# ade-ma/LibRedio

Measured on AMD Instinct MI355X. Metric: MSamples/s through FIR+FFT+resample chain, higher is better.
Workload: dtype f32

## Files before the change

__graft_entry__.py:

```python
import os
import subprocess
import sys

ROOT = os.path.dirname(os.path.abspath(__file__))
sys.path.insert(0, ROOT)


def build() -> None:
    import libredio_amd
    libredio_amd.build()
    libredio_amd.lib()
    libredio_amd.kisslib()
    import oracle
    oracle.build()
    oracle.lib()
    libredio_amd.samplerate_lib()
    subprocess.check_call(["make", "-C", os.path.join(ROOT, "tests", "emu"), "-s"])
    subprocess.check_call(["make", "-C", os.path.join(ROOT, "tests", "cpp"), "-s"])
    subprocess.check_call(["make", "-C", os.path.join(ROOT, "tests", "stub"), "-s"])
    subprocess.check_call(["make", "-C", os.path.join(ROOT, "tests", "cpp_src"), "-s"])
    subprocess.check_call(["make", "-C", os.path.join(ROOT, "tests", "emu_fftr"), "-s"])
    subprocess.check_call(["make", "-C", os.path.join(ROOT, "tests", "cpp_fftr"), "-s"])
    subprocess.check_call(["make", "-C", os.path.join(ROOT, "tests", "emu_ovsave_real"), "-s"])
    subprocess.check_call(["make", "-C", os.path.join(ROOT, "tests", "cpp_ovsave_real"), "-s"])
    subprocess.check_call(["make", "-C", os.path.join(ROOT, "tests", "emu_pspec"), "-s"])
    subprocess.check_call(["make", "-C", os.path.join(ROOT, "tests", "cpp_pspec"), "-s"])
    subprocess.check_call(["make", "-C", os.path.join(ROOT, "tests", "emu_pspec_u8"), "-s"])
    subprocess.check_call(["make", "-C", os.path.join(ROOT, "tests", "cpp_pspec_u8"), "-s"])
    subprocess.check_call(["make", "-C", os.path.join(ROOT, "tests", "emu_pspec_real"), "-s"])
    subprocess.check_call(["make", "-C", os.path.join(ROOT, "tests", "cpp_pspec_real"), "-s"])
    subprocess.check_call(["make", "-C", os.path.join(ROOT, "tests", "emu_pfb_pspec"), "-s"])
    subprocess.check_call(["make", "-C", os.path.join(ROOT, "tests", "cpp_pfb_pspec"), "-s"])
    subprocess.check_call(["make", "-C", os.path.join(ROOT, "tests", "emu_taps"), "-s"])
    subprocess.check_call(["make", "-C", os.path.join(ROOT, "tests", "emu_route"), "-s"])
    subprocess.check_call(["make", "-C", os.path.join(ROOT, "tests", "emu_sched"), "-s"])


def smoke() -> None:
    import numpy as np
    import torch
    import libredio_amd as R
    import oracle as O

    assert torch.cuda.is_available(), "smoke() needs a HIP device"
    torch.cuda.set_device(0)
    n = 8 * 1024 * 5 + 126
    taps = R.dsputils.lpf_corrected(127, 0.08)
    x = R.synth_iq(0x5EED0002, 0, n)
    xh = O.synth_iq(0x5EED0002, 0, n)
    assert np.array_equal(x.cpu().numpy().view(np.uint32), xh.view(np.uint32)), "device/host synthetic input differ"
    for fused in (True, False):
        chain = R.Chain(taps, 5, 1024, fused=fused)
        assert chain.is_fused
        got = chain(x).cpu().numpy()
        want = O.chain_fir_fft(xh, taps, 5, 1024, fused=fused)
        assert got.shape == want.shape == (8, 1024)
        assert np.array_equal(got.view(np.uint32), want.view(np.uint32)), f"chain (fused={fused}) differs from the oracle"
    print("smoke ok: fused FIR(127,/5)->FFT1024 chain is bit-identical to the oracle on 8 blocks")


if __name__ == "__main__":
    build()
    if len(sys.argv) > 1 and sys.argv[1] == "smoke":
        smoke()
```

libredio_amd/csrc/chain_v4.hip:

```cpp
#ifndef REDIO_EXP_CHAIN_NT
#define REDIO_EXP_CHAIN_NT 3
#endif
#ifndef REDIO_EXP_SEAM
#define REDIO_EXP_SEAM 15
#endif
#include "fir_core.h"
#include "fft_wave.h"
#include "redio_internal.h"
#include "../../include/redio.h"
#include <type_traits>

namespace redio {

typedef float v4f_t __attribute__((ext_vector_type(4)));

constexpr int chain_gcd(int a, int b) { return b == 0 ? a : chain_gcd(b, a % b); }

template <int N, typename F>
__device__ __forceinline__ void static_for4(F &&f)
{
    if constexpr (N > 0) {
        static_for4<N - 1>(f);
        f(std::integral_constant<int, N - 1>{});
    }
}

template <int K, int D, bool FUSED, int WPS, int CH, bool FIR_ONLY, bool TWP, bool IN_U8, bool PF2, bool RES, int SCH>
__device__ __forceinline__ void chain_v4_body(const float2 *__restrict__ x, const float *__restrict__ taps,
                                              const float2 *__restrict__ tw, float2 *__restrict__ out,
                                              long nblocks, long blocks_per_wave, long wave, unsigned long long *dbg, long dbg_cap)
{
    unsigned long long t0c = 0, t0r = 0;
    if (dbg) { t0c = __builtin_amdgcn_s_memtime(); t0r = __builtin_amdgcn_s_memrealtime(); }
    constexpr int R = 4;
    using G = FirGeomV<K, D, R>;
    constexpr int SUB_OUT = 64 * R;
    constexpr int SUB_NEW = SUB_OUT * D;
    constexpr int HALO = G::tile_in(SUB_OUT) - SUB_NEW;
    static_assert(HALO % 2 == 0 && SUB_NEW % 128 == 0 && 4 * SUB_OUT == 1024, "geometry");
    constexpr int HALO_V = HALO / 2;
    constexpr int NLD = SUB_NEW / 2 / 64;
    static_assert(HALO_V <= 64, "the halo moves with one instruction per lane");
    extern __shared__ __attribute__((aligned(16))) char smem[];
    v4f_t *xs4 = reinterpret_cast<v4f_t *>(smem);
    float2 *ex = reinterpret_cast<float2 *>(smem);

    const int lane = threadIdx.x;
    const long b0 = wave * blocks_per_wave;
    if (b0 >= nblocks) return;
    const long b1 = (b0 + blocks_per_wave < nblocks) ? b0 + blocks_per_wave : nblocks;
    const long nsub = 4 * (b1 - b0);
    typename std::conditional<RES, FirTapsResident<K>, FirNoResidentTaps>::type rtaps;
    if constexpr (RES) fir_taps_resident_load(rtaps, taps);
    using pair_t = typename std::conditional<IN_U8, unsigned, v4f_t>::type;
    [[maybe_unused]] const pair_t *src0 = (IN_U8 ? reinterpret_cast<const pair_t *>(reinterpret_cast<const unsigned *>(x) + b0 * 512 * (long)D)
                                : reinterpret_cast<const pair_t *>(x + b0 * 1024 * (long)D)) + lane;
    auto samples = [](pair_t w) -> v4f_t {
        if constexpr (IN_U8) return v4f_t{i2f(w & 255u), i2f((w >> 8) & 255u), i2f((w >> 16) & 255u), i2f(w >> 24)};
        else return w;
    };

    constexpr bool HOIST = (REDIO_EXP_SEAM & 1) != 0, BUF = PF2 || (REDIO_EXP_SEAM & 2) != 0, EARLY = (REDIO_EXP_SEAM & 4) != 0,
                   PRO = (REDIO_EXP_SEAM & 8) != 0;
    auto slot = [](int p) { return G::lds_index(2 * p) / 2; };
    constexpr int HSTR = G::LSTR / 2;
    static_assert((SUB_NEW / 2) % HSTR == 0, "a sub-tile is a whole number of lane strides");
    constexpr int HALO_DELTA = G::lds_index(SUB_NEW) / 2;
    constexpr int PER0 = G::PADN == 0 ? 1 : HSTR / chain_gcd(64, HSTR), PER = PER0 < NLD ? PER0 : NLD;
    constexpr int PARK_STEP = G::lds_index(2 * 64 * PER) / 2;
    static_assert(PER == NLD || (64 * PER) % HSTR == 0, "park slots repeat with period PER");
    auto halo_slots = [&](int lf, int &src, int &dst) {
        dst = slot(lf);
        if constexpr (EARLY) src = dst + (lf < HALO_V ? HALO_DELTA : 0);
        else src = slot(SUB_NEW / 2 + lf);
    };
    [[maybe_unused]] int park4[PER], hsrc4 = 0, hdst4 = 0;
    if constexpr (HOIST) {
        static_for4<PER>([&](auto I) { park4[I.value] = slot(HALO_V + lane + 64 * I.value); });
        halo_slots(lane, hsrc4, hdst4);
    }

    pair_t pre[NLD], pre2[PF2 ? NLD : 1];
    constexpr unsigned PB = sizeof(pair_t);
    constexpr int NT_LD = (REDIO_EXP_CHAIN_NT & 1) ? 2 : 0, NT_ST = (REDIO_EXP_CHAIN_NT & 2) ? 2 : 0;
    typedef unsigned v4u_t __attribute__((ext_vector_type(4)));
    typedef unsigned v2u_t __attribute__((ext_vector_type(2)));
    [[maybe_unused]] __amdgpu_buffer_rsrc_t ri, ro;
    if constexpr (BUF) {
        static_assert(!PF2 || !IN_U8, "PF2: cf32 input");
        const char *xb = reinterpret_cast<const char *>(x) + b0 * (512 * (long)D) * PB;
        ri = __builtin_amdgcn_make_buffer_rsrc(const_cast<char *>(xb), 0, (int)((HALO_V + nsub * (SUB_NEW / 2)) * PB), 0x00020000);
        ro = __builtin_amdgcn_make_buffer_rsrc(out + b0 * 1024, 0, (int)((b1 - b0) * 8192), 0x00020000);
    }
    [[maybe_unused]] auto buf_load = [&](unsigned vo, unsigned so, auto policy) -> pair_t {
        if constexpr (IN_U8) return __builtin_amdgcn_raw_buffer_load_b32(ri, vo, so, decltype(policy)::value);
        else return __builtin_bit_cast(v4f_t, __builtin_amdgcn_raw_buffer_load_b128(ri, vo, so, decltype(policy)::value));
    };
    auto fetch_to = [&](pair_t(&dst)[NLD], long j) {
        if constexpr (BUF) {
            const unsigned sub = (unsigned)((HALO_V + j * (SUB_NEW / 2)) * PB);
            const unsigned vo = PB * (unsigned)lane + (PF2 ? sub : 0u), so = PF2 ? 0u : sub;
            static_for4<NLD>([&](auto I) {
                constexpr unsigned off = 64u * PB * I.value, imm = off % 4096u;
                dst[I.value] = buf_load(vo + imm, so + (off - imm), std::integral_constant<int, NT_LD>{});
                if constexpr (!PF2) __builtin_amdgcn_sched_barrier(0);
            });
        } else {
            const pair_t *src = src0 + HALO_V + j * (SUB_NEW / 2);
#if REDIO_EXP_CHAIN_NT & 1
            static_for4<NLD>([&](auto I) { dst[I.value] = __builtin_nontemporal_load(src + 64 * I.value); });
#else
            static_for4<NLD>([&](auto I) { dst[I.value] = src[64 * I.value]; });
#endif
        }
    };
    auto park_from = [&](pair_t(&from)[NLD]) {
#if REDIO_EXP_ABLATE == 3
#pragma unroll
        for (int i = 0; i < NLD; ++i) { pair_t keep = from[i]; asm volatile("" : : "v"(keep)); }
#else
        static_for4<NLD>([&](auto I) {
            constexpr int i = I.value;
            if constexpr (HOIST) xs4[park4[i % PER] + (i / PER) * PARK_STEP] = samples(from[i]);
            else xs4[G::lds_index(HALO + 2 * (lane + 64 * i)) / 2] = samples(from[i]);
        });
#endif
    };
    [[maybe_unused]] auto store_block = [&](const float2(&a)[16], long blk, int ln) {
        if constexpr (BUF) {
            const unsigned so = (unsigned)(blk * 8192);
            static_for4<16>([&](auto I) {
                constexpr unsigned k0 = I.value / 4, k1 = I.value % 4;
                const float2 v = a[k1 + 4 * k0];
                __builtin_amdgcn_raw_buffer_store_b64(v2u_t{__builtin_bit_cast(unsigned, v.x), __builtin_bit_cast(unsigned, v.y)}, ro,
                                                      8u * (unsigned)ln + (512u * k1 + 2048u * (k0 & 1)), so + 4096u * (k0 >> 1), NT_ST);
            });
        } else fft1kn_store_spectrum(a, out + (b0 + blk) * 1024, ln);
    };

    static_assert(SCH == 0 || (!PF2 && !FIR_ONLY && TWP && WPS == 2), "the block schedules: the transforming product forms");
    constexpr int EXH_OFF = G::lds_elems(SUB_OUT) > FFT1KN_LDS ? G::lds_elems(SUB_OUT) : FFT1KN_LDS;
    constexpr int T12_OFF = EXH_OFF + (SCH == 2 ? FFT1KN_HALF_LDS : 0);
    constexpr bool TABLE = (PF2 || SCH != 0) && !FIR_ONLY;
    static_assert(!TABLE || (T12_OFF + 64) * sizeof(float2) <= 160 * 1024 / 8 - 480, "within the request of chain_v4_lds at two waves per SIMD");
    auto table_index = [](int l) {
        const int k4 = l / 15, i = l % 15;
        return i < 3 ? 64 * k4 * (i + 1) : 16 * (k4 + 4 * ((i - 3) / 3)) * ((i - 3) % 3 + 1);
    };
    Fft1knTw34 t34;
    [[maybe_unused]] float2 one = make_float2(0.f, 0.f);
    if constexpr (PRO) {
        pair_t head;
        if constexpr (BUF) head = buf_load(PB * (unsigned)lane, 0u, std::integral_constant<int, 0>{});
        else head = src0[0];
        fetch_to(pre, 0);
        [[maybe_unused]] float2 twv = make_float2(0.f, 0.f);
        if constexpr (TABLE) twv = tw[table_index(lane < 60 ? lane : 0)];
        if (!FIR_ONLY && TWP) fft1kn_load_tw34(t34, lane, tw);
        if constexpr (SCH != 0) one = tw[0];
        xs4[slot(lane)] = samples(head);
        if constexpr (TABLE) ex[T12_OFF + lane] = twv;
        park_from(pre);
        wave_lds_fence();
    } else {
        if (lane < HALO_V) {
            if constexpr (BUF) xs4[slot(lane)] = samples(buf_load(PB * (unsigned)lane, 0u, std::integral_constant<int, 0>{}));
            else xs4[slot(lane)] = samples(src0[0]);
        }
        if constexpr (TABLE)
            if (lane < 60) ex[T12_OFF + lane] = tw[table_index(lane)];
        fetch_to(pre, 0);
        park_from(pre);
        wave_lds_fence();
        if (!FIR_ONLY && TWP) fft1kn_load_tw34(t34, lane, tw);
        if constexpr (SCH != 0) one = tw[0];
    }
    if constexpr (SCH != 0) asm volatile("" : "+v"(one.x), "+v"(one.y));

    float2 a[16];
    if constexpr (!(PRO && SCH == 1)) {
#pragma unroll
        for (int i = 0; i < 16; ++i) a[i] = make_float2(0.f, 0.f);
    }
    constexpr int NCH = fir_num_chunks<K, D, R, CH>();
    struct Seam { int lf, hs, hd; v4f_t halo; };
    auto fir = [&](Seam &s, float2(&acc)[R], auto &&hook) {
        s.lf = lane, s.hs = hsrc4, s.hd = hdst4, s.halo = v4f_t{0.f, 0.f, 0.f, 0.f};
        if constexpr (!HOIST) {
            asm volatile("" : "+v"(s.lf));
            if constexpr (EARLY) halo_slots(s.lf, s.hs, s.hd);
        }
        auto hk = [&](auto C) {
            if constexpr (EARLY && decltype(C)::value == NCH - 1) s.halo = xs4[s.hs];
            hook(C);
        };
        if constexpr (RES) fir_lane_v_res<K, D, R, FUSED, CH>(xs4, s.lf, rtaps, acc, hk);
        else fir_lane_v<K, D, R, FUSED, CH>(xs4, s.lf, taps, acc, hk);
    };
    auto halo_read = [&](Seam &s, bool more) {
        if constexpr (!EARLY) {
            if constexpr (!HOIST) halo_slots(s.lf, s.hs, s.hd);
            if (more && s.lf < HALO_V) s.halo = xs4[s.hs];
        }
    };
    auto halo_write = [&](const Seam &s) {
        if constexpr (EARLY) xs4[s.hd] = s.halo;
        else if (s.lf < HALO_V) xs4[HOIST ? s.hd : slot(s.lf)] = s.halo;
    };
    auto transform_lane = [&]() {
        int ln = lane;
        if constexpr (!HOIST) asm volatile("" : "+v"(ln));
        return ln;
    };
    auto step = [&](long j, auto ahead, auto place, pair_t(&req)[NLD], pair_t(&parked)[NLD]) {
        constexpr int AHEAD = decltype(ahead)::value, S = decltype(place)::value;
        const bool more = S >= 0 || j + 1 < nsub;
        if (S >= 0 || j + AHEAD < nsub) fetch_to(req, j + AHEAD);
        float2 acc[R];
#pragma unroll
        for (int r = 0; r < R; ++r) acc[r] = make_float2(0.f, 0.f);
        Seam seam;
        fir(seam, acc, FirNoHook{});
        if (FIR_ONLY) {
            const v4f_t y0 = v4f_t{acc[0].x, acc[0].y, acc[1].x, acc[1].y}, y1 = v4f_t{acc[2].x, acc[2].y, acc[3].x, acc[3].y};
            if constexpr (BUF) {
                const unsigned so = (unsigned)(j * (SUB_OUT * 8));
                __builtin_amdgcn_raw_buffer_store_b128(__builtin_bit_cast(v4u_t, y0), ro, 32u * (unsigned)lane, so, 0);
                __builtin_amdgcn_raw_buffer_store_b128(__builtin_bit_cast(v4u_t, y1), ro, 32u * (unsigned)lane + 16u, so, 0);
            } else {
                v4f_t *y4 = reinterpret_cast<v4f_t *>(out + (b0 * 4 + j) * SUB_OUT) + 2 * lane;
                y4[0] = y0;
                y4[1] = y1;
            }
        } else {
#pragma unroll
            for (int i = 0; i < 12; ++i) a[i] = a[i + 4];
#pragma unroll
            for (int r = 0; r < R; ++r) a[12 + r] = acc[r];
        }
        wave_lds_fence();
        halo_read(seam, more);
        if (!FIR_ONLY && (S == 3 || (S < 0 && (j & 3) == 3))) {
            wave_lds_fence();
            const int ln = transform_lane();
            Fft1knTw12 t12;
            if constexpr (PF2) {
                const float2 *T = ex + T12_OFF + 15 * (ln >> 4);
#pragma unroll
                for (int i = 0; i < 3; ++i) t12.a[i] = T[i];
#pragma unroll
                for (int i = 0; i < 12; ++i) t12.b[i] = T[3 + i];
            } else fft1kn_load_tw12(t12, ln, tw);
            if (!TWP) fft1kn_load_tw34(t34, ln, tw);
            fft1kn_wave_regs<false>(a, ex, tw, t12, t34, ln);
            store_block(a, j >> 2, ln);
            wave_lds_fence();
        }
        if (more) {
            halo_write(seam);
            park_from(parked);
        }
        wave_lds_fence();
    };
    [[maybe_unused]] auto t12_lds = [&](Fft1knTw12 &t12, int ln) {
        const float2 *T = ex + T12_OFF + 15 * (ln >> 4);
#pragma unroll
        for (int i = 0; i < 3; ++i) t12.a[i] = T[i];
#pragma unroll
        for (int i = 0; i < 12; ++i) t12.b[i] = T[3 + i];
    };
    [[maybe_unused]] auto sstep = [&](long j, auto place, bool more_, bool xform_, auto &&hook) {
        constexpr int S = decltype(place)::value;
        const bool more = S < 3 || more_, xform = S == 3 && xform_;
        if (more) fetch_to(pre, j + 1);
        float2 acc[R];
#pragma unroll
        for (int r = 0; r < R; ++r) acc[r] = make_float2(0.f, 0.f);
        Seam seam;
        fir(seam, acc, hook);
#pragma unroll
        for (int r = 0; r < R; ++r) a[4 * S + r] = acc[r];
        wave_lds_fence();
        halo_read(seam, more);
        if (xform) {
            wave_lds_fence();
            const int ln = transform_lane();
            Fft1knTw12 t12;
            t12_lds(t12, ln);
            const float2 one1[1] = {one};
            fft1kn_wave_regs<false>(a, ex, one1, t12, t34, ln);
            store_block(a, j >> 2, ln);
            wave_lds_fence();
        }
        if (more) {
            halo_write(seam);
            park_from(pre);
        }
        wave_lds_fence();
    };
    using S0 = std::integral_constant<int, 0>;
    using S1 = std::integral_constant<int, 1>;
    using S2 = std::integral_constant<int, 2>;
    using S3 = std::integral_constant<int, 3>;
    if constexpr (SCH == 1) {
        const long nb = b1 - b0;
#pragma unroll 1
        for (long blk = 0; blk < nb; ++blk) {
            sstep(4 * blk, S0{}, true, false, FirNoHook{});
            sstep(4 * blk + 1, S1{}, true, false, FirNoHook{});
            sstep(4 * blk + 2, S2{}, true, false, FirNoHook{});
            sstep(4 * blk + 3, S3{}, blk + 1 < nb, true, FirNoHook{});
        }
    } else if constexpr (SCH == 2) {
        const long nb = b1 - b0;
        sstep(0, S0{}, true, false, FirNoHook{});
#pragma unroll 1
        for (long blk = 0;; ++blk) {
            sstep(4 * blk + 1, S1{}, true, false, FirNoHook{});
            sstep(4 * blk + 2, S2{}, true, false, FirNoHook{});
            const bool more = blk + 1 < nb;
            sstep(4 * blk + 3, S3{}, more, !more, FirNoHook{});
            if (!more) break;
            float2 ap[16], u[16];
#pragma unroll
            for (int i = 0; i < 16; ++i) ap[i] = a[i];
            int ln = lane;
            asm volatile("" : "+v"(ln));
            Fft1knTw12 t12;
            float2 *dst = out + (b0 + blk) * 1024;
            auto piece = [&](auto C) {
                fft1kn_wave_piece<decltype(C)::value, false>(ap, u, ex + EXH_OFF, one, ex + T12_OFF + 15 * (ln >> 4), t12, t34, dst, ln);
            };
            sstep(4 * blk + 4, S0{}, true, false, piece);
            if constexpr (NCH < FFT1KN_PIECES)
                static_for4<FFT1KN_PIECES - NCH>([&](auto I) { piece(std::integral_constant<int, NCH + I.value>{}); });
        }
    } else if constexpr (PF2) {
        fetch_to(pre, 1);
        using two = std::integral_constant<int, 2>;
#pragma unroll 1
        for (long j = 0; j < nsub; j += 4) {
            step(j, two{}, std::integral_constant<int, 0>{}, pre2, pre);
            step(j + 1, two{}, std::integral_constant<int, 1>{}, pre, pre2);
            step(j + 2, two{}, std::integral_constant<int, 2>{}, pre2, pre);
            step(j + 3, two{}, std::integral_constant<int, 3>{}, pre, pre2);
        }
    } else {
#pragma unroll 1
        for (long j = 0; j < nsub; ++j) step(j, std::integral_constant<int, 1>{}, std::integral_constant<int, -1>{}, pre, pre);
    }
    if (dbg && lane == 0 && (long)blockIdx.x < dbg_cap) {
        dbg[4 * blockIdx.x] = __builtin_amdgcn_s_memtime() - t0c;
        dbg[4 * blockIdx.x + 1] = __builtin_amdgcn_s_memrealtime() - t0r;
        dbg[4 * blockIdx.x + 2] = t0r;
        unsigned xcc = 0;
        asm volatile("s_getreg_b32 %0, hwreg(HW_REG_XCC_ID)" : "=s"(xcc));
        unsigned hwid = 0;
        asm volatile("s_getreg_b32 %0, hwreg(HW_REG_HW_ID)" : "=s"(hwid));
        dbg[4 * blockIdx.x + 3] = ((unsigned long long)xcc << 32) | hwid;
    }
}

template <int WPS, bool FIR_ONLY, bool TWP, bool PF2, bool RES>
constexpr int chain_v4_sched()
{
    return (WPS == 2 && !FIR_ONLY && TWP && !PF2) ? 1 : 0;
}

template <int K, int D, bool FUSED, int WPS, int CH, bool FIR_ONLY = false, bool TWP = false, bool IN_U8 = false, bool PF2 = false>
__global__ __launch_bounds__(64, WPS) void chain_v4_kernel(const float2 *__restrict__ x, const float *__restrict__ taps,
                                                           const float2 *__restrict__ tw, float2 *__restrict__ out,
                                                           long nblocks, long blocks_per_wave, unsigned long long *dbg, long dbg_cap)
{
    chain_v4_body<K, D, FUSED, WPS, CH, FIR_ONLY, TWP, IN_U8, PF2, true, chain_v4_sched<WPS, FIR_ONLY, TWP, PF2, true>()>(x, taps, tw, out, nblocks, blocks_per_wave, (long)blockIdx.x, dbg, dbg_cap);
}
template <int K, int D, bool FUSED, int WPS, int CH, bool FIR_ONLY = false, bool TWP = false, bool IN_U8 = false, bool PF2 = false>
__global__ __launch_bounds__(64, WPS) void chain_v4_anytaps_kernel(const float2 *__restrict__ x, const float *__restrict__ taps,
                                                                   const float2 *__restrict__ tw, float2 *__restrict__ out,
                                                                   long nblocks, long blocks_per_wave, unsigned long long *dbg, long dbg_cap)
{
    chain_v4_body<K, D, FUSED, WPS, CH, FIR_ONLY, TWP, IN_U8, PF2, false, chain_v4_sched<WPS, FIR_ONLY, TWP, PF2, false>()>(x, taps, tw, out, nblocks, blocks_per_wave, (long)blockIdx.x, dbg, dbg_cap);
}

#ifdef REDIO_MEASURE
template <int K, int D, bool FUSED>
__global__ __launch_bounds__(64, 2) void chain_v4_sched2_kernel(const float2 *__restrict__ x, const float *__restrict__ taps,
                                                                const float2 *__restrict__ tw, float2 *__restrict__ out,
                                                                long nblocks, long blocks_per_wave, unsigned long long *dbg, long dbg_cap)
{
    chain_v4_body<K, D, FUSED, 2, 8, false, true, false, false, true, 2>(x, taps, tw, out, nblocks, blocks_per_wave, (long)blockIdx.x, dbg, dbg_cap);
}
#endif

struct ChainList {
    const float2 *x[REDIO_LIST_MAX];
    float2 *out[REDIO_LIST_MAX];
    long nblocks[REDIO_LIST_MAX];
    unsigned wave0[REDIO_LIST_MAX + 1];
    int count;
};

template <int K, int D, bool FUSED, bool RES>
__device__ __forceinline__ void chain_v4_list_body(const ChainList &list, const float *__restrict__ taps, const float2 *__restrict__ tw,
                                                   long blocks_per_wave)
{
    const unsigned w = blockIdx.x;
    int m = 0;
    for (int i = 1; i < list.count; ++i) m = w >= list.wave0[i] ? i : m;
    m = __builtin_amdgcn_readfirstlane(m);
    chain_v4_body<K, D, FUSED, 2, 8, false, true, false, false, RES, chain_v4_sched<2, false, true, false, RES>()>(list.x[m], taps, tw, list.out[m], list.nblocks[m], blocks_per_wave,
                                                                     (long)(w - list.wave0[m]), nullptr, 0);
}

template <int K, int D, bool FUSED>
__global__ __launch_bounds__(64, 2) void chain_v4_list_kernel(const ChainList list, const float *__restrict__ taps,
                                                              const float2 *__restrict__ tw, long blocks_per_wave)
{
    chain_v4_list_body<K, D, FUSED, true>(list, taps, tw, blocks_per_wave);
}
template <int K, int D, bool FUSED>
__global__ __launch_bounds__(64, 2) void chain_v4_anytaps_list_kernel(const ChainList list, const float *__restrict__ taps,
                                                                      const float2 *__restrict__ tw, long blocks_per_wave)
{
    chain_v4_list_body<K, D, FUSED, false>(list, taps, tw, blocks_per_wave);
}

long chain_v4_blocks_per_wave(long nblocks, int WPS)
{
    long waves = 4L * WPS * num_cus();
    if (waves > nblocks) waves = nblocks;
    if (waves < 1) waves = 1;
    long bpw = nblocks / (6 * waves);
    if (bpw < 1) bpw = 1;
    if (bpw > 4) bpw = 4;
    if (const char *e = measure_env("REDIO_CHAIN_BPW")) { const long v = atol(e); if (v >= 1) bpw = v; }
    return bpw;
}

template <int K, int D, int WPS, bool PF2 = false>
static constexpr size_t chain_v4_lds()
{
    static_assert(WPS == 2 || WPS == 3, "two wavefronts per SIMD (the chain: its transform needs 197 registers) or three (the FIR alone: 94-145)");
    using G = FirGeomV<K, D, 4>;
    constexpr int ELEMS = (G::lds_elems(256) > FFT1KN_LDS ? G::lds_elems(256) : FFT1KN_LDS) + (PF2 ? 64 : 0);
    constexpr size_t LDS_NEED = (size_t)ELEMS * sizeof(float2);
    static_assert(4 * WPS * LDS_NEED <= 160 * 1024, "4*WPS waves per CU");
    constexpr size_t LDS = (160 * 1024 / (4 * WPS)) - 480 > LDS_NEED ? (160 * 1024 / (4 * WPS)) - 480 : LDS_NEED;
    static_assert((4 * WPS + 1) * LDS > 160 * 1024, "one more wave must not fit");
    return LDS;
}

template <int K, int D, int WPS, int CH, bool FIR_ONLY = false, bool TWP = false, bool IN_U8 = false, bool PF2 = false>
static hipError_t launch_v4_t(const float2 *x, const float *taps, bool pal, const float2 *tw, float2 *out, long nblocks, bool fused,
                              hipStream_t s, unsigned long long *dbg, long dbg_cap = 0)
{
    constexpr size_t LDS = chain_v4_lds<K, D, WPS, PF2>();
    const long bpw = chain_v4_blocks_per_wave(nblocks, WPS);
    const long grid = (nblocks + bpw - 1) / bpw;
    if (pal) {
        if (fused) hipLaunchKernelGGL((chain_v4_kernel<K, D, true, WPS, CH, FIR_ONLY, TWP, IN_U8, PF2>), dim3((unsigned)grid), dim3(64), LDS, s, x, taps, tw, out, nblocks, bpw, dbg, dbg_cap);
        else hipLaunchKernelGGL((chain_v4_kernel<K, D, false, WPS, CH, FIR_ONLY, TWP, IN_U8, PF2>), dim3((unsigned)grid), dim3(64), LDS, s, x, taps, tw, out, nblocks, bpw, dbg, dbg_cap);
    } else {
        if (fused) hipLaunchKernelGGL((chain_v4_anytaps_kernel<K, D, true, WPS, CH, FIR_ONLY, TWP, IN_U8, PF2>), dim3((unsigned)grid), dim3(64), LDS, s, x, taps, tw, out, nblocks, bpw, dbg, dbg_cap);
        else hipLaunchKernelGGL((chain_v4_anytaps_kernel<K, D, false, WPS, CH, FIR_ONLY, TWP, IN_U8, PF2>), dim3((unsigned)grid), dim3(64), LDS, s, x, taps, tw, out, nblocks, bpw, dbg, dbg_cap);
    }
    return hipGetLastError();
}

hipError_t launch_chain_v4(const float2 *x, const float *taps, bool pal, const float2 *tw, float2 *out, long nblocks, bool fused,
                           hipStream_t s, unsigned long long *dbg, long dbg_cap)
{
#ifdef REDIO_MEASURE
    if (measure_env("REDIO_CHAIN_WPS3")) return launch_v4_t<127, 5, 3, 8, false, false>(x, taps, pal, tw, out, nblocks, fused, s, dbg, dbg_cap);
    if (measure_env("REDIO_CHAIN_PF2")) return launch_v4_t<127, 5, 2, 8, false, true, false, true>(x, taps, pal, tw, out, nblocks, fused, s, dbg, dbg_cap);
    if (pal && measure_env("REDIO_CHAIN_SCHED2")) {
        const long bpw = chain_v4_blocks_per_wave(nblocks, 2);
        const dim3 grid((unsigned)((nblocks + bpw - 1) / bpw));
        if (fused) hipLaunchKernelGGL((chain_v4_sched2_kernel<127, 5, true>), grid, dim3(64), (chain_v4_lds<127, 5, 2>()), s, x, taps, tw, out, nblocks, bpw, dbg, dbg_cap);
        else hipLaunchKernelGGL((chain_v4_sched2_kernel<127, 5, false>), grid, dim3(64), (chain_v4_lds<127, 5, 2>()), s, x, taps, tw, out, nblocks, bpw, dbg, dbg_cap);
        return hipGetLastError();
    }
#endif
    return launch_v4_t<127, 5, 2, 8, false, true>(x, taps, pal, tw, out, nblocks, fused, s, dbg, dbg_cap);
}

hipError_t launch_chain_v4_u8(const void *bytes, const float *taps, bool pal, const float2 *tw, float2 *out, long nblocks, bool fused, hipStream_t s)
{
    return launch_v4_t<127, 5, 2, 8, false, true, true>((const float2 *)bytes, taps, pal, tw, out, nblocks, fused, s, nullptr);
}

hipError_t launch_chain_v4_shape_u8(int K, int D, const void *bytes, const float *taps, bool pal, const float2 *tw, float2 *out, long nblocks, bool fused,
                                    hipStream_t s)
{
    const float2 *x = (const float2 *)bytes;
    if (K == 63 && D == 5) return launch_v4_t<63, 5, 2, 8, false, true, true>(x, taps, pal, tw, out, nblocks, fused, s, nullptr);
    if (K == 127 && D == 1) return launch_v4_t<127, 1, 2, 8, false, true, true>(x, taps, pal, tw, out, nblocks, fused, s, nullptr);
    if (K == 63 && D == 1) return launch_v4_t<63, 1, 2, 8, false, true, true>(x, taps, pal, tw, out, nblocks, fused, s, nullptr);
    if (K == 127 && D == 3) return launch_v4_t<127, 3, 2, 8, false, true, true>(x, taps, pal, tw, out, nblocks, fused, s, nullptr);
    return hipErrorNotSupported;
}

hipError_t launch_chain_v4_shape(int K, int D, const float2 *x, const float *taps, bool pal, const float2 *tw, float2 *out, long nblocks, bool fused,
                                 hipStream_t s)
{
    if (K == 63 && D == 5) return launch_v4_t<63, 5, 2, 8, false, true>(x, taps, pal, tw, out, nblocks, fused, s, nullptr);
    if (K == 127 && D == 1) return launch_v4_t<127, 1, 2, 8, false, true>(x, taps, pal, tw, out, nblocks, fused, s, nullptr);
    if (K == 63 && D == 1) return launch_v4_t<63, 1, 2, 8, false, true>(x, taps, pal, tw, out, nblocks, fused, s, nullptr);
    if (K == 127 && D == 3) return launch_v4_t<127, 3, 2, 8, false, true>(x, taps, pal, tw, out, nblocks, fused, s, nullptr);
    return hipErrorNotSupported;
}

template <int K, int D>
static hipError_t launch_v4_list_t(const float2 *const *x, float2 *const *out, const long *nblocks, int count, const float *taps,
                                   bool pal, const float2 *tw, bool fused, hipStream_t s)
{
    ChainList list;
    long total = 0;
    for (int i = 0; i < count; ++i) total += nblocks[i];
    const long bpw = chain_v4_blocks_per_wave(total, 2);
    unsigned w = 0;
    for (int i = 0; i < count; ++i) {
        list.x[i] = x[i];
        list.out[i] = out[i];
        list.nblocks[i] = nblocks[i];
        list.wave0[i] = w;
        w += (unsigned)((nblocks[i] + bpw - 1) / bpw);
    }
    list.wave0[count] = w;
    list.count = count;
    constexpr size_t LDS = chain_v4_lds<K, D, 2>();
    if (pal) {
        if (fused) hipLaunchKernelGGL((chain_v4_list_kernel<K, D, true>), dim3(w), dim3(64), LDS, s, list, taps, tw, bpw);
        else hipLaunchKernelGGL((chain_v4_list_kernel<K, D, false>), dim3(w), dim3(64), LDS, s, list, taps, tw, bpw);
    } else {
        if (fused) hipLaunchKernelGGL((chain_v4_anytaps_list_kernel<K, D, true>), dim3(w), dim3(64), LDS, s, list, taps, tw, bpw);
        else hipLaunchKernelGGL((chain_v4_anytaps_list_kernel<K, D, false>), dim3(w), dim3(64), LDS, s, list, taps, tw, bpw);
    }
    return hipGetLastError();
}

hipError_t launch_chain_list(int K, long D, const float2 *const *x, float2 *const *out, const long *nblocks, int count, const float *taps,
                             bool pal, const float2 *tw, bool fused, hipStream_t s)
{
    if (count < 1 || count > REDIO_LIST_MAX) return hipErrorInvalidValue;
    for (int i = 0; i < count; ++i)
        if (nblocks[i] < 1 || (reinterpret_cast<uintptr_t>(x[i]) & 15) != 0) return hipErrorInvalidValue;
    if (K == 127 && D == 5) return launch_v4_list_t<127, 5>(x, out, nblocks, count, taps, pal, tw, fused, s);
    if (K == 127 && D == 3) return launch_v4_list_t<127, 3>(x, out, nblocks, count, taps, pal, tw, fused, s);
    if (K == 127 && D == 1) return launch_v4_list_t<127, 1>(x, out, nblocks, count, taps, pal, tw, fused, s);
    if (K == 63 && D == 5) return launch_v4_list_t<63, 5>(x, out, nblocks, count, taps, pal, tw, fused, s);
    if (K == 63 && D == 1) return launch_v4_list_t<63, 1>(x, out, nblocks, count, taps, pal, tw, fused, s);
    return hipErrorNotSupported;
}

hipError_t launch_fir_v4(int K, int D, const float2 *x, const float *taps, bool pal, float2 *y, long nblocks, bool fused, hipStream_t s)
{
    if (!measure_env("REDIO_FIR_WPS2")) {
        if (K == 127 && D == 5) return launch_v4_t<127, 5, 3, 8, true>(x, taps, pal, nullptr, y, nblocks, fused, s, nullptr);
        if (K == 63 && D == 5) return launch_v4_t<63, 5, 3, 8, true>(x, taps, pal, nullptr, y, nblocks, fused, s, nullptr);
        if (K == 63 && D == 1) return launch_v4_t<63, 1, 3, 8, true>(x, taps, pal, nullptr, y, nblocks, fused, s, nullptr);
        if (K == 127 && D == 3) return launch_v4_t<127, 3, 3, 8, true>(x, taps, pal, nullptr, y, nblocks, fused, s, nullptr);
    }
#ifdef REDIO_MEASURE
    if (K == 127 && D == 5) return launch_v4_t<127, 5, 2, 8, true>(x, taps, pal, nullptr, y, nblocks, fused, s, nullptr);
    if (K == 63 && D == 5) return launch_v4_t<63, 5, 2, 8, true>(x, taps, pal, nullptr, y, nblocks, fused, s, nullptr);
    if (K == 63 && D == 1) return launch_v4_t<63, 1, 2, 8, true>(x, taps, pal, nullptr, y, nblocks, fused, s, nullptr);
#endif
    return hipErrorNotSupported;
}

}
```

Baseline: 538,400.

## Align streamed input loads to cache lines by shifting the halo split

Adds a ChainGeom helper and a new default seam mode (31) that computes, per wave, how many extra pairs to fold into the halo so the body loads start on a 128-byte line. The buffer resource is rebased on the aligned address, halo and park LDS slots are shifted by that amount, and the head and tail loads use separate resources so the ends stay in bounds. The goal is to avoid loads that straddle cache lines in the streaming FIR input. In exchange it adds per-wave address arithmetic, an extra resource build on the tail load, and a larger LDS image.

```diff
diff --git a/__graft_entry__.py b/__graft_entry__.py
--- a/__graft_entry__.py
+++ b/__graft_entry__.py
@@ -34,6 +34,7 @@
     subprocess.check_call(["make", "-C", os.path.join(ROOT, "tests", "emu_taps"), "-s"])
     subprocess.check_call(["make", "-C", os.path.join(ROOT, "tests", "emu_route"), "-s"])
     subprocess.check_call(["make", "-C", os.path.join(ROOT, "tests", "emu_sched"), "-s"])
+    subprocess.check_call(["make", "-C", os.path.join(ROOT, "tests", "emu_chain"), "-s"])
 
 
 def smoke() -> None:
diff --git a/libredio_amd/csrc/chain_core.h b/libredio_amd/csrc/chain_core.h
--- /dev/null
+++ b/libredio_amd/csrc/chain_core.h
@@ -0,0 +1,56 @@
+#pragma once
+#include "fir_core.h"
+
+namespace redio {
+
+constexpr int chain_gcd(int a, int b) { return b == 0 ? a : chain_gcd(b, a % b); }
+
+template <int K, int D, bool IN_U8>
+struct ChainGeom {
+    static constexpr int R = 4;
+    using G = FirGeomV<K, D, R>;
+    static constexpr int SUB_OUT = 64 * R;
+    static constexpr int SUB_NEW = SUB_OUT * D;
+    static constexpr int HALO = G::tile_in(SUB_OUT) - SUB_NEW;
+    static_assert(HALO % 2 == 0 && SUB_NEW % 128 == 0, "geometry");
+    static constexpr int HALO_V = HALO / 2;
+    static constexpr int NLD = SUB_NEW / 2 / 64;
+    static_assert(HALO_V <= 64, "the halo moves with one instruction per lane");
+    static constexpr unsigned PB = IN_U8 ? 4 : 16;
+    static constexpr unsigned LINE = 128;
+
+    RD_HD static constexpr int extra(unsigned long long run_addr)
+    {
+        const unsigned need = (LINE - (unsigned)((run_addr + PB * HALO_V) % LINE)) % LINE;
+        const int e = (int)(need / PB);
+        return (need % PB == 0 && HALO_V + e <= 64) ? e : 0;
+    }
+
+    RD_HD static constexpr int slot(int p) { return G::lds_index(2 * p) / 2; }
+    static constexpr int IMG_PAIRS = 64 + SUB_NEW / 2;
+    static constexpr int IMG_ELEMS = (G::lds_index(2 * IMG_PAIRS - 1) + 2) & ~1;
+
+    static constexpr int HSTR = G::LSTR / 2;
+    static_assert((SUB_NEW / 2) % HSTR == 0, "a sub-tile is a whole number of lane strides");
+    static constexpr int HALO_DELTA = G::lds_index(SUB_NEW) / 2;
+    static constexpr int PER0 = G::PADN == 0 ? 1 : HSTR / chain_gcd(64, HSTR), PER = PER0 < NLD ? PER0 : NLD;
+    static constexpr int PARK_STEP = G::lds_index(2 * 64 * PER) / 2;
+    static_assert(PER == NLD || (64 * PER) % HSTR == 0, "park slots repeat with period PER");
+
+    RD_HD static constexpr int park_slot(int e, int lane, int i) { return slot(HALO_V + e + lane + 64 * i); }
+    RD_HD static constexpr void halo_slots(int e, int lf, int &src, int &dst)
+    {
+        dst = slot(lf);
+        src = dst + (lf < HALO_V + e ? HALO_DELTA : 0);
+    }
+
+    RD_HD static constexpr long body_start(int e) { return (long)PB * e; }
+    RD_HD static constexpr long sub_offset(long j) { return (HALO_V + j * (SUB_NEW / 2)) * (long)PB; }
+    RD_HD static constexpr unsigned load_offset(int i) { return 64u * PB * (unsigned)i; }
+    RD_HD static constexpr unsigned load_imm(int i) { return load_offset(i) % 4096u; }
+    RD_HD static constexpr long run_bytes(long nsub) { return (HALO_V + nsub * (SUB_NEW / 2)) * (long)PB; }
+    RD_HD static constexpr long body_bytes(int e, long nsub) { return run_bytes(nsub) - body_start(e); }
+    RD_HD static constexpr long tail_advance(long nsub) { return sub_offset(nsub - 1) + (long)(load_offset(NLD - 1) - load_imm(NLD - 1)); }
+};
+
+}
diff --git a/libredio_amd/csrc/chain_v4.hip b/libredio_amd/csrc/chain_v4.hip
--- a/libredio_amd/csrc/chain_v4.hip
+++ b/libredio_amd/csrc/chain_v4.hip
@@ -2,9 +2,9 @@
 #define REDIO_EXP_CHAIN_NT 3
 #endif
 #ifndef REDIO_EXP_SEAM
-#define REDIO_EXP_SEAM 15
-#endif
-#include "fir_core.h"
+#define REDIO_EXP_SEAM 31
+#endif
+#include "chain_core.h"
 #include "fft_wave.h"
 #include "redio_internal.h"
 #include "../../include/redio.h"
@@ -14,8 +14,6 @@
 
 typedef float v4f_t __attribute__((ext_vector_type(4)));
 
-constexpr int chain_gcd(int a, int b) { return b == 0 ? a : chain_gcd(b, a % b); }
-
 template <int N, typename F>
 __device__ __forceinline__ void static_for4(F &&f)
 {
@@ -32,15 +30,15 @@
 {
     unsigned long long t0c = 0, t0r = 0;
     if (dbg) { t0c = __builtin_amdgcn_s_memtime(); t0r = __builtin_amdgcn_s_memrealtime(); }
-    constexpr int R = 4;
+    using CG = ChainGeom<K, D, IN_U8>;
+    constexpr int R = CG::R;
     using G = FirGeomV<K, D, R>;
-    constexpr int SUB_OUT = 64 * R;
-    constexpr int SUB_NEW = SUB_OUT * D;
-    constexpr int HALO = G::tile_in(SUB_OUT) - SUB_NEW;
-    static_assert(HALO % 2 == 0 && SUB_NEW % 128 == 0 && 4 * SUB_OUT == 1024, "geometry");
-    constexpr int HALO_V = HALO / 2;
-    constexpr int NLD = SUB_NEW / 2 / 64;
-    static_assert(HALO_V <= 64, "the halo moves with one instruction per lane");
+    constexpr int SUB_OUT = CG::SUB_OUT;
+    constexpr int SUB_NEW = CG::SUB_NEW;
+    constexpr int HALO = CG::HALO;
+    static_assert(4 * SUB_OUT == 1024, "geometry");
+    constexpr int HALO_V = CG::HALO_V;
+    constexpr int NLD = CG::NLD;
     extern __shared__ __attribute__((aligned(16))) char smem[];
     v4f_t *xs4 = reinterpret_cast<v4f_t *>(smem);
     float2 *ex = reinterpret_cast<float2 *>(smem);
@@ -61,48 +59,50 @@
     };
 
     constexpr bool HOIST = (REDIO_EXP_SEAM & 1) != 0, BUF = PF2 || (REDIO_EXP_SEAM & 2) != 0, EARLY = (REDIO_EXP_SEAM & 4) != 0,
-                   PRO = (REDIO_EXP_SEAM & 8) != 0;
-    auto slot = [](int p) { return G::lds_index(2 * p) / 2; };
-    constexpr int HSTR = G::LSTR / 2;
-    static_assert((SUB_NEW / 2) % HSTR == 0, "a sub-tile is a whole number of lane strides");
-    constexpr int HALO_DELTA = G::lds_index(SUB_NEW) / 2;
-    constexpr int PER0 = G::PADN == 0 ? 1 : HSTR / chain_gcd(64, HSTR), PER = PER0 < NLD ? PER0 : NLD;
-    constexpr int PARK_STEP = G::lds_index(2 * 64 * PER) / 2;
-    static_assert(PER == NLD || (64 * PER) % HSTR == 0, "park slots repeat with period PER");
+                   PRO = (REDIO_EXP_SEAM & 8) != 0, ALIGN = (REDIO_EXP_SEAM & 31) == 31;
+    constexpr unsigned PB = CG::PB;
+    const char *xb = reinterpret_cast<const char *>(x) + b0 * (512 * (long)D) * PB;
+    const int e = ALIGN ? CG::extra(reinterpret_cast<uintptr_t>(xb)) : 0;
+    const char *xe = reinterpret_cast<const char *>((reinterpret_cast<uintptr_t>(xb) + (unsigned)e * PB) & 0xffffffffffffull);
+    auto slot = [](int p) { return CG::slot(p); };
+    constexpr int PER = CG::PER, PARK_STEP = CG::PARK_STEP;
     auto halo_slots = [&](int lf, int &src, int &dst) {
-        dst = slot(lf);
-        if constexpr (EARLY) src = dst + (lf < HALO_V ? HALO_DELTA : 0);
-        else src = slot(SUB_NEW / 2 + lf);
+        if constexpr (EARLY) CG::halo_slots(e, lf, src, dst);
+        else dst = slot(lf), src = slot(SUB_NEW / 2 + lf);
     };
     [[maybe_unused]] int park4[PER], hsrc4 = 0, hdst4 = 0;
     if constexpr (HOIST) {
-        static_for4<PER>([&](auto I) { park4[I.value] = slot(HALO_V + lane + 64 * I.value); });
+        static_for4<PER>([&](auto I) { park4[I.value] = CG::park_slot(e, lane, I.value); });
         halo_slots(lane, hsrc4, hdst4);
     }
 
     pair_t pre[NLD], pre2[PF2 ? NLD : 1];
-    constexpr unsigned PB = sizeof(pair_t);
+    static_assert(PB == sizeof(pair_t), "a pair in the stream");
     constexpr int NT_LD = (REDIO_EXP_CHAIN_NT & 1) ? 2 : 0, NT_ST = (REDIO_EXP_CHAIN_NT & 2) ? 2 : 0;
     typedef unsigned v4u_t __attribute__((ext_vector_type(4)));
     typedef unsigned v2u_t __attribute__((ext_vector_type(2)));
     [[maybe_unused]] __amdgpu_buffer_rsrc_t ri, ro;
     if constexpr (BUF) {
         static_assert(!PF2 || !IN_U8, "PF2: cf32 input");
-        const char *xb = reinterpret_cast<const char *>(x) + b0 * (512 * (long)D) * PB;
-        ri = __builtin_amdgcn_make_buffer_rsrc(const_cast<char *>(xb), 0, (int)((HALO_V + nsub * (SUB_NEW / 2)) * PB), 0x00020000);
+        ri = __builtin_amdgcn_make_buffer_rsrc(const_cast<char *>(xe), 0, (int)CG::body_bytes(e, nsub), 0x00020000);
         ro = __builtin_amdgcn_make_buffer_rsrc(out + b0 * 1024, 0, (int)((b1 - b0) * 8192), 0x00020000);
     }
-    [[maybe_unused]] auto buf_load = [&](unsigned vo, unsigned so, auto policy) -> pair_t {
-        if constexpr (IN_U8) return __builtin_amdgcn_raw_buffer_load_b32(ri, vo, so, decltype(policy)::value);
-        else return __builtin_bit_cast(v4f_t, __builtin_amdgcn_raw_buffer_load_b128(ri, vo, so, decltype(policy)::value));
-    };
-    auto fetch_to = [&](pair_t(&dst)[NLD], long j) {
+    [[maybe_unused]] auto buf_load_of = [&](__amdgpu_buffer_rsrc_t r, unsigned vo, unsigned so, auto policy) -> pair_t {
+        if constexpr (IN_U8) return __builtin_amdgcn_raw_buffer_load_b32(r, vo, so, decltype(policy)::value);
+        else return __builtin_bit_cast(v4f_t, __builtin_amdgcn_raw_buffer_load_b128(r, vo, so, decltype(policy)::value));
+    };
+    [[maybe_unused]] auto buf_load = [&](unsigned vo, unsigned so, auto policy) -> pair_t { return buf_load_of(ri, vo, so, policy); };
+    auto fetch_to = [&](pair_t(&dst)[NLD], long j, auto maybe_tail) {
         if constexpr (BUF) {
-            const unsigned sub = (unsigned)((HALO_V + j * (SUB_NEW / 2)) * PB);
+            const unsigned sub = (unsigned)CG::sub_offset(j);
             const unsigned vo = PB * (unsigned)lane + (PF2 ? sub : 0u), so = PF2 ? 0u : sub;
             static_for4<NLD>([&](auto I) {
-                constexpr unsigned off = 64u * PB * I.value, imm = off % 4096u;
-                dst[I.value] = buf_load(vo + imm, so + (off - imm), std::integral_constant<int, NT_LD>{});
+                constexpr unsigned off = CG::load_offset(I.value), imm = CG::load_imm(I.value);
+                if constexpr (ALIGN && !PF2 && I.value == NLD - 1 && decltype(maybe_tail)::value) {
+                    const unsigned adv = j == nsub - 1 ? so + (off - imm) : 0u;
+                    const __amdgpu_buffer_rsrc_t r = __builtin_amdgcn_make_buffer_rsrc(const_cast<char *>(xe) + adv, 0, (int)(CG::body_bytes(e, nsub) - adv), 0x00020000);
+                    dst[I.value] = buf_load_of(r, vo + imm, so + (off - imm) - adv, std::integral_constant<int, NT_LD>{});
+                } else dst[I.value] = buf_load(vo + imm, so + (off - imm), std::integral_constant<int, NT_LD>{});
                 if constexpr (!PF2) __builtin_amdgcn_sched_barrier(0);
             });
         } else {
@@ -139,7 +139,9 @@
     };
 
     static_assert(SCH == 0 || (!PF2 && !FIR_ONLY && TWP && WPS == 2), "the block schedules: the transforming product forms");
-    constexpr int EXH_OFF = G::lds_elems(SUB_OUT) > FFT1KN_LDS ? G::lds_elems(SUB_OUT) : FFT1KN_LDS;
+    constexpr int IMG = ALIGN ? CG::IMG_ELEMS : G::lds_elems(SUB_OUT);
+    static_assert(IMG * sizeof(float2) <= 160 * 1024 / (4 * WPS) - 480, "the image within the request of chain_v4_lds");
+    constexpr int EXH_OFF = IMG > FFT1KN_LDS ? IMG : FFT1KN_LDS;
     constexpr int T12_OFF = EXH_OFF + (SCH == 2 ? FFT1KN_HALF_LDS : 0);
     constexpr bool TABLE = (PF2 || SCH != 0) && !FIR_ONLY;
     static_assert(!TABLE || (T12_OFF + 64) * sizeof(float2) <= 160 * 1024 / 8 - 480, "within the request of chain_v4_lds at two waves per SIMD");
@@ -151,9 +153,11 @@
     [[maybe_unused]] float2 one = make_float2(0.f, 0.f);
     if constexpr (PRO) {
         pair_t head;
-        if constexpr (BUF) head = buf_load(PB * (unsigned)lane, 0u, std::integral_constant<int, 0>{});
+        if constexpr (ALIGN)
+            head = buf_load_of(__builtin_amdgcn_make_buffer_rsrc(const_cast<char *>(xb), 0, (int)(64 * PB), 0x00020000), PB * (unsigned)lane, 0u, std::integral_constant<int, 0>{});
+        else if constexpr (BUF) head = buf_load(PB * (unsigned)lane, 0u, std::integral_constant<int, 0>{});
         else head = src0[0];
-        fetch_to(pre, 0);
+        fetch_to(pre, 0, std::false_type{});
         [[maybe_unused]] float2 twv = make_float2(0.f, 0.f);
         if constexpr (TABLE) twv = tw[table_index(lane < 60 ? lane : 0)];
         if (!FIR_ONLY && TWP) fft1kn_load_tw34(t34, lane, tw);
@@ -169,7 +173,7 @@
         }
         if constexpr (TABLE)
             if (lane < 60) ex[T12_OFF + lane] = tw[table_index(lane)];
-        fetch_to(pre, 0);
+        fetch_to(pre, 0, std::false_type{});
         park_from(pre);
         wave_lds_fence();
         if (!FIR_ONLY && TWP) fft1kn_load_tw34(t34, lane, tw);
@@ -215,7 +219,7 @@
     auto step = [&](long j, auto ahead, auto place, pair_t(&req)[NLD], pair_t(&parked)[NLD]) {
         constexpr int AHEAD = decltype(ahead)::value, S = decltype(place)::value;
         const bool more = S >= 0 || j + 1 < nsub;
-        if (S >= 0 || j + AHEAD < nsub) fetch_to(req, j + AHEAD);
+        if (S >= 0 || j + AHEAD < nsub) fetch_to(req, j + AHEAD, std::true_type{});
         float2 acc[R];
 #pragma unroll
         for (int r = 0; r < R; ++r) acc[r] = make_float2(0.f, 0.f);
@@ -272,7 +276,7 @@
     [[maybe_unused]] auto sstep = [&](long j, auto place, bool more_, bool xform_, auto &&hook) {
         constexpr int S = decltype(place)::value;
         const bool more = S < 3 || more_, xform = S == 3 && xform_;
-        if (more) fetch_to(pre, j + 1);
+        if (more) fetch_to(pre, j + 1, std::integral_constant<bool, S == 2>{});
         float2 acc[R];
 #pragma unroll
         for (int r = 0; r < R; ++r) acc[r] = make_float2(0.f, 0.f);
@@ -336,7 +340,7 @@
                 static_for4<FFT1KN_PIECES - NCH>([&](auto I) { piece(std::integral_constant<int, NCH + I.value>{}); });
         }
     } else if constexpr (PF2) {
-        fetch_to(pre, 1);
+        fetch_to(pre, 1, std::true_type{});
         using two = std::integral_constant<int, 2>;
 #pragma unroll 1
         for (long j = 0; j < nsub; j += 4) {
```

Result: no change. 544,400 (median of 6 runs) (+1.1%).
